# feiyeha/EGM-Unet

Hardware: AMD Instinct MI355X
Metric: train images/sec at 3x512x512 bs=8/GPU (higher is better)
Workload: dtype bf16; 1 GPU; EGM-UNet GRFBUNet(3,2,base_c=32) fwd+5-term-loss+bwd+SGD, 8x3x512x512 per GPU (BASELINE.json configs[1]); global_batch=8, parallelism=dp1, launch=hipGraph replay, world_size=1

## Files before the change

### egm_unet_amd/csrc/blocks.hip

```cpp
#include "common.h"

namespace {

inline int stream_grid(long long total_threads) {
    long long b = (total_threads + 255) / 256;
    if (b > 256 * 16) b = 256 * 16;
    if (b < 1) b = 1;
    return (int)b;
}
__device__ __forceinline__ float sigm(float v) { return 1.f / (1.f + expf(-v)); }

#define PIX_LOOP(total_expr)                                                                           \
    const int ncv = C >> 3;                                                                            \
    const long long total = (total_expr);                                                              \
    for (long long i = blockIdx.x * 256LL + threadIdx.x; i < total; i += (long long)gridDim.x * 256)
#define PIX_LOOP_XCD(total_expr)                                                                       \
    const int ncv = C >> 3;                                                                            \
    const long long total = (total_expr);                                                              \
    for (long long i = xcd_contiguous_item(blockIdx.x, gridDim.x) * 256LL + threadIdx.x; i < total; i += (long long)gridDim.x * 256)

template <typename T>
__global__ void highpass3_kernel(const T* __restrict__ x, int ldx, T* __restrict__ out, int ldo, int N, int H, int W, int C) {
    PIX_LOOP_XCD((long long)N * H * W * ncv) {
        long long p; int cv; egm_divmod(i, ncv, p, cv);
        int xx, yy; egm_pix_yx(p, H, W, yy, xx);
        float s[8], c[8], v[8];
        zero8(s);
        load8(x + p * ldx + cv * 8, c);
#pragma unroll
        for (int r = -1; r <= 1; ++r)
#pragma unroll
            for (int q = -1; q <= 1; ++q) {
                if (yy + r < 0 || yy + r >= H || xx + q < 0 || xx + q >= W) continue;
                load8(x + (p + (long long)r * W + q) * ldx + cv * 8, v);
#pragma unroll
                for (int j = 0; j < 8; ++j) s[j] += v[j];
            }
#pragma unroll
        for (int j = 0; j < 8; ++j) c[j] -= s[j] * (1.f / 9.f);
        store8(out + p * ldo + cv * 8, c);
    }
}

template <typename T>
__global__ void gate_mul_fwd_kernel(const T* __restrict__ x, int ldx, const T* __restrict__ w, int ldw, T* __restrict__ out, int ldo,
                                    long long npix, int C) {
    PIX_LOOP(npix * ncv) {
        long long p; int cv; egm_divmod(i, ncv, p, cv);
        float a[8], b[8];
        load8(x + p * ldx + cv * 8, a); load8(w + p * ldw + cv * 8, b);
#pragma unroll
        for (int j = 0; j < 8; ++j) a[j] *= (1.f + b[j]);
        store8(out + p * ldo + cv * 8, a);
    }
}
template <typename T>
__global__ void gate_mul_bwd_kernel(const T* __restrict__ g, int ldg, const T* __restrict__ x, int ldx, const T* __restrict__ w, int ldw,
                                    T* __restrict__ dx, int lddx, T* __restrict__ dw, int lddw, long long npix, int C) {
    PIX_LOOP(npix * ncv) {
        long long p; int cv; egm_divmod(i, ncv, p, cv);
        float gg[8], a[8], b[8], o1[8], o2[8];
        load8(g + p * ldg + cv * 8, gg); load8(x + p * ldx + cv * 8, a); load8(w + p * ldw + cv * 8, b);
#pragma unroll
        for (int j = 0; j < 8; ++j) { o1[j] = gg[j] * (1.f + b[j]); o2[j] = gg[j] * a[j]; }
        store8(dx + p * lddx + cv * 8, o1); store8(dw + p * lddw + cv * 8, o2);
    }
}

template <typename T>
__global__ void scale_add_relu_fwd_kernel(const T* __restrict__ a, int lda, float alpha, const T* __restrict__ b, int ldb,
                                          T* __restrict__ out, int ldo, long long npix, int C) {
    PIX_LOOP(npix * ncv) {
        long long p; int cv; egm_divmod(i, ncv, p, cv);
        float u[8], v[8];
        load8(a + p * lda + cv * 8, u); load8(b + p * ldb + cv * 8, v);
#pragma unroll
        for (int j = 0; j < 8; ++j) u[j] = fmaxf(fmaf(alpha, u[j], v[j]), 0.f);
        store8(out + p * ldo + cv * 8, u);
    }
}
template <typename T>
__global__ void scale_add_relu_bwd_kernel(const T* __restrict__ g, int ldg, const T* __restrict__ out, int ldo, float alpha,
                                          T* __restrict__ da, int ldda, T* __restrict__ db, int lddb, long long npix, int C) {
    PIX_LOOP(npix * ncv) {
        long long p; int cv; egm_divmod(i, ncv, p, cv);
        float gg[8], o[8], u[8];
        load8(g + p * ldg + cv * 8, gg); load8(out + p * ldo + cv * 8, o);
#pragma unroll
        for (int j = 0; j < 8; ++j) { gg[j] = o[j] > 0.f ? gg[j] : 0.f; u[j] = alpha * gg[j]; }
        store8(da + p * ldda + cv * 8, u); store8(db + p * lddb + cv * 8, gg);
    }
}

template <int GROUP>
// ... 588 lines not shown
        const T v = from_f32<T>(red[((long long)n * 2) * C + c]);
        dst[(long long)n * ldd + c] = v;
        dst[(long long)(N + n) * ldd + c] = v;
    }
}

template <typename T>
__global__ void fold2_pack_kernel(const float* __restrict__ w, float* __restrict__ out, T* __restrict__ wf, T* __restrict__ wd, int rows, int K,
                                  int CoutP, int CinP) {
    for (int i = blockIdx.x * blockDim.x + threadIdx.x; i < CoutP * CinP; i += gridDim.x * blockDim.x) {
        const int co = i / CinP, ci = i - co * CinP;
        float v = 0.f;
        if (co < rows && ci < K) {
            v = w[(long long)co * 2 * K + ci] + w[(long long)co * 2 * K + K + ci];
            out[co * K + ci] = v;
        }
        wf[i] = from_f32<T>(v);
        wd[(long long)ci * CoutP + co] = from_f32<T>(v);
    }
}
template <typename T>
__global__ void merge357_pack_kernel(const float* __restrict__ w3, const float* __restrict__ w5, const float* __restrict__ w7,
                                     const float* __restrict__ b3, const float* __restrict__ b5, const float* __restrict__ b7,
                                     float* __restrict__ w, float* __restrict__ b, T* __restrict__ wf, T* __restrict__ wd, int Co, int Ci,
                                     int CoutP, int CinP) {
    const int total = 49 * CoutP * CinP;
    for (int i = blockIdx.x * blockDim.x + threadIdx.x; i < total; i += gridDim.x * blockDim.x) {
        const int ci = i % CinP, co = (i / CinP) % CoutP, t = i / (CinP * CoutP), r = t / 7, sx = t % 7;
        float v = 0.f;
        if (co < Co && ci < Ci) {
            const int oc = co * Ci + ci;
            v = w7[oc * 49 + t];
            if (r >= 1 && r <= 5 && sx >= 1 && sx <= 5) v += w5[oc * 25 + (r - 1) * 5 + (sx - 1)];
            if (r >= 2 && r <= 4 && sx >= 2 && sx <= 4) v += w3[oc * 9 + (r - 2) * 3 + (sx - 2)];
            w[oc * 49 + t] = v;
        }
        wf[i] = from_f32<T>(v);
        wd[((long long)(48 - t) * CinP + ci) * CoutP + co] = from_f32<T>(v);
        if (i < Co) b[i] = b3[i] + b5[i] + b7[i];
    }
}

}

#define EGM_REQ_VEC(name, ptr, ld, C)                                                                      \
    EGM_REQUIRE((ptr) != nullptr && egm_aligned16(ptr) && (C) > 0 && (C) % 8 == 0 && (ld) >= (C) && (ld) % 8 == 0, \
                name ": bad tensor (ptr/alignment/C=%d/ld=%d)", (int)(C), (int)(ld))
#define EGM_GROUP_SWITCH(G, ...)                                                                \
    switch (G) { case 1: { constexpr int GROUP = 1; __VA_ARGS__; break; } case 2: { constexpr int GROUP = 2; __VA_ARGS__; break; } \
                 case 4: { constexpr int GROUP = 4; __VA_ARGS__; break; } case 8: { constexpr int GROUP = 8; __VA_ARGS__; break; } \
                 case 16: { constexpr int GROUP = 16; __VA_ARGS__; break; } case 32: { constexpr int GROUP = 32; __VA_ARGS__; break; } \
                 default: { constexpr int GROUP = 64; __VA_ARGS__; break; } }

extern "C" int egm_highpass3(int dtype, const void* x, int ldx, void* out, int ldo, int N, int H, int W, int C, egm_stream_t s) {
    EGM_REQ_VEC("highpass3", x, ldx, C); EGM_REQ_VEC("highpass3", out, ldo, C);
    EGM_REQUIRE(N > 0 && H > 0 && W > 0, "highpass3: bad shape");
    EGM_DISPATCH_DTYPE(dtype, hipLaunchKernelGGL((highpass3_kernel<T>), dim3(stream_grid((long long)N * H * W * (C / 8))), dim3(256), 0,
                                                 (hipStream_t)s, (const T*)x, ldx, (T*)out, ldo, N, H, W, C));
    EGM_CHECK_LAUNCH("highpass3");
    return EGM_OK;
}
extern "C" int egm_gate_mul_fwd(int dtype, const void* x, int ldx, const void* w, int ldw, void* out, int ldo, long long npix, int C,
                                egm_stream_t s) {
    EGM_REQ_VEC("gate_mul_fwd", x, ldx, C); EGM_REQ_VEC("gate_mul_fwd", w, ldw, C); EGM_REQ_VEC("gate_mul_fwd", out, ldo, C);
    EGM_DISPATCH_DTYPE(dtype, hipLaunchKernelGGL((gate_mul_fwd_kernel<T>), dim3(stream_grid(npix * (C / 8))), dim3(256), 0, (hipStream_t)s,
                                                 (const T*)x, ldx, (const T*)w, ldw, (T*)out, ldo, npix, C));
    EGM_CHECK_LAUNCH("gate_mul_fwd");
    return EGM_OK;
}
extern "C" int egm_gate_mul_bwd(int dtype, const void* g, int ldg, const void* x, int ldx, const void* w, int ldw, void* dx, int lddx,
                                void* dw, int lddw, long long npix, int C, egm_stream_t s) {
    EGM_REQ_VEC("gate_mul_bwd", g, ldg, C); EGM_REQ_VEC("gate_mul_bwd", x, ldx, C); EGM_REQ_VEC("gate_mul_bwd", w, ldw, C);
    EGM_REQ_VEC("gate_mul_bwd", dx, lddx, C); EGM_REQ_VEC("gate_mul_bwd", dw, lddw, C);
    EGM_DISPATCH_DTYPE(dtype, hipLaunchKernelGGL((gate_mul_bwd_kernel<T>), dim3(stream_grid(npix * (C / 8))), dim3(256), 0, (hipStream_t)s,
                                                 (const T*)g, ldg, (const T*)x, ldx, (const T*)w, ldw, (T*)dx, lddx, (T*)dw, lddw, npix, C));
    EGM_CHECK_LAUNCH("gate_mul_bwd");
    return EGM_OK;
}
extern "C" int egm_scale_add_relu_fwd(int dtype, const void* a, int lda, float alpha, const void* b, int ldb, void* out, int ldo,
                                      long long npix, int C, egm_stream_t s) {
    EGM_REQ_VEC("scale_add_relu_fwd", a, lda, C); EGM_REQ_VEC("scale_add_relu_fwd", b, ldb, C); EGM_REQ_VEC("scale_add_relu_fwd", out, ldo, C);
    EGM_DISPATCH_DTYPE(dtype, hipLaunchKernelGGL((scale_add_relu_fwd_kernel<T>), dim3(stream_grid(npix * (C / 8))), dim3(256), 0,
                                                 (hipStream_t)s, (const T*)a, lda, alpha, (const T*)b, ldb, (T*)out, ldo, npix, C));
    EGM_CHECK_LAUNCH("scale_add_relu_fwd");
    return EGM_OK;
}
extern "C" int egm_scale_add_relu_bwd(int dtype, const void* g, int ldg, const void* out, int ldo, float alpha, void* da, int ldda,
                                      void* db, int lddb, long long npix, int C, egm_stream_t s) {
    EGM_REQ_VEC("scale_add_relu_bwd", g, ldg, C); EGM_REQ_VEC("scale_add_relu_bwd", out, ldo, C);
    EGM_REQ_VEC("scale_add_relu_bwd", da, ldda, C); EGM_REQ_VEC("scale_add_relu_bwd", db, lddb, C);
    EGM_DISPATCH_DTYPE(dtype, hipLaunchKernelGGL((scale_add_relu_bwd_kernel<T>), dim3(stream_grid(npix * (C / 8))), dim3(256), 0,
                                                 (hipStream_t)s, (const T*)g, ldg, (const T*)out, ldo, alpha, (T*)da, ldda, (T*)db, lddb, npix, C));
    EGM_CHECK_LAUNCH("scale_add_relu_bwd");
    return EGM_OK;
}
extern "C" int egm_gate3_fwd(int dtype, const void* x, int ldx, const void* t, int ldt, void* out, int ldo, long long npix, int C,
                             egm_stream_t s) {
    EGM_REQ_VEC("gate3_fwd", x, ldx, C); EGM_REQ_VEC("gate3_fwd", t, ldt, 8); EGM_REQ_VEC("gate3_fwd", out, ldo, C);
    EGM_DISPATCH_DTYPE(dtype, hipLaunchKernelGGL((gate3_fwd_kernel<T>), dim3(stream_grid(npix * (C / 8))), dim3(256), 0, (hipStream_t)s,
                                                 (const T*)x, ldx, (const T*)t, ldt, (T*)out, ldo, npix, C));
    EGM_CHECK_LAUNCH("gate3_fwd");
    return EGM_OK;
}
extern "C" int egm_gate3_bwd(int dtype, const void* g, int ldg, const void* x, int ldx, const void* t, int ldt, void* dx, int lddx,
                             void* dt, int lddt, long long npix, int C, egm_stream_t s) {
    EGM_REQ_VEC("gate3_bwd", g, ldg, C); EGM_REQ_VEC("gate3_bwd", x, ldx, C); EGM_REQ_VEC("gate3_bwd", t, ldt, 8);
    EGM_REQ_VEC("gate3_bwd", dx, lddx, C); EGM_REQ_VEC("gate3_bwd", dt, lddt, 8);
    const int G = group_for(C / 8 > 64 ? 64 : C / 8);
    const int grid = stream_grid(npix * G);
// ... 236 lines not shown
```

### egm_unet_amd/csrc/pool_up.hip

```cpp
#include "common.h"

namespace {

inline int stream_grid(long long total_threads) {
    long long b = (total_threads + 255) / 256;
    if (b > 256 * 16) b = 256 * 16;
    if (b < 1) b = 1;
    return (int)b;
}

template <typename T>
__global__ void nchw_to_nhwc_kernel(const float* __restrict__ src, T* __restrict__ dst, int ld, int N, int C, long long HW) {
    const long long total = (long long)N * HW;
    for (long long i = blockIdx.x * 256LL + threadIdx.x; i < total; i += (long long)gridDim.x * 256) {
        const long long n = i / HW, p = i - n * HW;
        for (int c0 = 0; c0 < ld; c0 += 8) {
            float v[8];
#pragma unroll
            for (int j = 0; j < 8; ++j) v[j] = (c0 + j < C) ? src[(n * C + c0 + j) * HW + p] : 0.f;
            store8(dst + i * ld + c0, v);
        }
    }
}
template <typename T>
__global__ void nhwc_to_nchw_kernel(const T* __restrict__ src, int ld, float* __restrict__ dst, int N, int C, long long HW) {
    const long long total = (long long)N * HW;
    for (long long i = blockIdx.x * 256LL + threadIdx.x; i < total; i += (long long)gridDim.x * 256) {
        const long long n = i / HW, p = i - n * HW;
        for (int c0 = 0; c0 < C; c0 += 8) {
            float v[8];
            load8(src + i * ld + c0, v);
#pragma unroll
            for (int j = 0; j < 8; ++j) if (c0 + j < C) dst[(n * C + c0 + j) * HW + p] = v[j];
        }
    }
}

template <typename T>
__global__ void maxpool2_fwd_kernel(const T* __restrict__ x, int ldx, T* __restrict__ y, int ldy, int N, int H, int W, int C) {
    const int ncv = C >> 3, Ho = H >> 1, Wo = W >> 1;
    const long long total = (long long)N * Ho * Wo * ncv;
    for (long long i = blockIdx.x * 256LL + threadIdx.x; i < total; i += (long long)gridDim.x * 256) {
        long long p; int cv; egm_divmod(i, ncv, p, cv);
        int n, oy, ox; egm_pix_nyx(p, Ho, Wo, n, oy, ox);
        const T* b = x + (((long long)n * H + 2 * oy) * W + 2 * ox) * ldx + cv * 8;
        float a[8], v[8];
        load8(b, a);
        load8(b + ldx, v);
#pragma unroll
        for (int j = 0; j < 8; ++j) a[j] = fmaxf(a[j], v[j]);
        load8(b + (long long)W * ldx, v);
#pragma unroll
        for (int j = 0; j < 8; ++j) a[j] = fmaxf(a[j], v[j]);
// ... 387 lines not shown
        load8(a + p * lda + cv * 8, v);
        load8(b + p * ldb + cv * 8, u);
#pragma unroll
        for (int j = 0; j < 8; ++j) v[j] += u[j];
        load8(c + p * ldc + cv * 8, u);
#pragma unroll
        for (int j = 0; j < 8; ++j) v[j] += u[j];
        if (d != nullptr) {
            load8(d + p * ldd + cv * 8, u);
#pragma unroll
            for (int j = 0; j < 8; ++j) v[j] += u[j];
        }
        store8(out + p * ldo + cv * 8, v);
    }
}
template <typename T>
__global__ void sum4_hp_kernel(const T* __restrict__ a, int lda, const T* __restrict__ b, int ldb, const T* __restrict__ c, int ldc,
                               const T* __restrict__ d, int ldd, T* __restrict__ out, int ldo, int N, int H, int W, int C) {
    const int ncv = C >> 3;
    const long long total = (long long)N * H * W * ncv;
    for (long long i = xcd_contiguous_item(blockIdx.x, gridDim.x) * 256LL + threadIdx.x; i < total; i += (long long)gridDim.x * 256) {
        long long p; int cv; egm_divmod(i, ncv, p, cv);
        int xx, yy; egm_pix_yx(p, H, W, yy, xx);
        float v[8], u[8], s8[8];
        zero8(s8);
        load8(a + p * lda + cv * 8, v);
#pragma unroll
        for (int r = -1; r <= 1; ++r)
#pragma unroll
            for (int q = -1; q <= 1; ++q) {
                if (yy + r < 0 || yy + r >= H || xx + q < 0 || xx + q >= W) continue;
                load8(a + (p + (long long)r * W + q) * lda + cv * 8, u);
#pragma unroll
                for (int j = 0; j < 8; ++j) s8[j] += u[j];
            }
#pragma unroll
        for (int j = 0; j < 8; ++j) v[j] = to_f32(from_f32<T>(v[j] - s8[j] * (1.f / 9.f)));
        load8(b + p * ldb + cv * 8, u);
#pragma unroll
        for (int j = 0; j < 8; ++j) v[j] += u[j];
        if (c != nullptr) {
            load8(c + p * ldc + cv * 8, u);
#pragma unroll
            for (int j = 0; j < 8; ++j) v[j] += u[j];
        }
        if (d != nullptr) {
            load8(d + p * ldd + cv * 8, u);
#pragma unroll
            for (int j = 0; j < 8; ++j) v[j] += u[j];
        }
        store8(out + p * ldo + cv * 8, v);
    }
}
__global__ void vec_add_f32_kernel(float* __restrict__ y, const float* __restrict__ x, long long n) {
    for (long long i = blockIdx.x * 256LL + threadIdx.x; i < n; i += (long long)gridDim.x * 256) y[i] += x[i];
}
__global__ void fill_f32_kernel(float* __restrict__ y, float v, long long n) {
    for (long long i = blockIdx.x * 256LL + threadIdx.x; i < n; i += (long long)gridDim.x * 256) y[i] = v;
}

}

#define EGM_REQ_VEC(name, ptr, ld, C)                                                                      \
    EGM_REQUIRE((ptr) != nullptr && egm_aligned16(ptr) && (C) > 0 && (C) % 8 == 0 && (ld) >= (C) && (ld) % 8 == 0, \
                name ": bad tensor (ptr/alignment/C=%d/ld=%d)", (int)(C), (int)(ld))

extern "C" int egm_nchw_to_nhwc(int dtype, const void* src, void* dst, int ld, int N, int C, int H, int W, egm_stream_t s) {
    EGM_REQUIRE(src && dst && egm_aligned16(dst) && N > 0 && C > 0 && H > 0 && W > 0 && ld >= C && ld % 8 == 0, "nchw_to_nhwc: bad args");
    const long long HW = (long long)H * W;
    EGM_DISPATCH_DTYPE(dtype, hipLaunchKernelGGL((nchw_to_nhwc_kernel<T>), dim3(stream_grid(N * HW)), dim3(256), 0, (hipStream_t)s,
                                                 (const float*)src, (T*)dst, ld, N, C, HW));
    EGM_CHECK_LAUNCH("nchw_to_nhwc");
    return EGM_OK;
}
extern "C" int egm_nhwc_to_nchw(int dtype, const void* src, int ld, void* dst, int N, int C, int H, int W, egm_stream_t s) {
    EGM_REQUIRE(src && dst && egm_aligned16(src) && N > 0 && C > 0 && H > 0 && W > 0 && ld >= C && ld % 8 == 0, "nhwc_to_nchw: bad args");
    const long long HW = (long long)H * W;
    EGM_DISPATCH_DTYPE(dtype, hipLaunchKernelGGL((nhwc_to_nchw_kernel<T>), dim3(stream_grid(N * HW)), dim3(256), 0, (hipStream_t)s,
                                                 (const T*)src, ld, (float*)dst, N, C, HW));
    EGM_CHECK_LAUNCH("nhwc_to_nchw");
    return EGM_OK;
}

extern "C" int egm_maxpool2_fwd(int dtype, const void* x, int ldx, void* y, int ldy, int N, int H, int W, int C, egm_stream_t s) {
    EGM_REQ_VEC("maxpool2_fwd", x, ldx, C);
    EGM_REQ_VEC("maxpool2_fwd", y, ldy, C);
    EGM_REQUIRE(N > 0 && H >= 2 && W >= 2, "maxpool2_fwd: bad shape");
    const long long total = (long long)N * (H / 2) * (W / 2) * (C / 8);
    EGM_DISPATCH_DTYPE(dtype, hipLaunchKernelGGL((maxpool2_fwd_kernel<T>), dim3(stream_grid(total)), dim3(256), 0, (hipStream_t)s,
                                                 (const T*)x, ldx, (T*)y, ldy, N, H, W, C));
    EGM_CHECK_LAUNCH("maxpool2_fwd");
    return EGM_OK;
}
extern "C" int egm_maxpool2_bwd(int dtype, const void* x, int ldx, const void* dy, int lddy, void* dx, int lddx, int N, int H, int W,
                                int C, egm_stream_t s) {
    EGM_REQ_VEC("maxpool2_bwd", x, ldx, C);
    EGM_REQ_VEC("maxpool2_bwd", dy, lddy, C);
    EGM_REQ_VEC("maxpool2_bwd", dx, lddx, C);
    EGM_REQUIRE(N > 0 && H >= 2 && W >= 2, "maxpool2_bwd: bad shape");
    const long long total = (long long)N * (H / 2) * (W / 2) * (C / 8);
    EGM_DISPATCH_DTYPE(dtype, {
        hipLaunchKernelGGL((maxpool2_bwd_kernel<T>), dim3(stream_grid(total)), dim3(256), 0, (hipStream_t)s, (const T*)x, ldx,
                           (const T*)dy, lddy, (const T*)nullptr, 0, (T*)dx, lddx, N, H, W, C);
        if ((H & 1) || (W & 1))
            hipLaunchKernelGGL((zero_tail_kernel<T>), dim3(stream_grid((long long)N * H * W * (C / 8))), dim3(256), 0, (hipStream_t)s,
                               (T*)dx, lddx, N, H, W, C);
    });
    EGM_CHECK_LAUNCH("maxpool2_bwd");
    return EGM_OK;
}

extern "C" int egm_maxpool2_bwd_add(int dtype, const void* x, int ldx, const void* dy, int lddy, const void* add, int ldadd, void* dx, int lddx,
                                    int N, int H, int W, int C, egm_stream_t s) {
    EGM_REQ_VEC("maxpool2_bwd_add", x, ldx, C); EGM_REQ_VEC("maxpool2_bwd_add", dy, lddy, C); EGM_REQ_VEC("maxpool2_bwd_add", add, ldadd, C);
    EGM_REQ_VEC("maxpool2_bwd_add", dx, lddx, C);
    EGM_REQUIRE(N > 0 && H >= 2 && W >= 2 && !(H & 1) && !(W & 1), "maxpool2_bwd_add: H and W must be even (got %d x %d)", H, W);
    const long long total = (long long)N * (H / 2) * (W / 2) * (C / 8);
    EGM_DISPATCH_DTYPE(dtype, hipLaunchKernelGGL((maxpool2_bwd_kernel<T>), dim3(stream_grid(total)), dim3(256), 0, (hipStream_t)s, (const T*)x, ldx,
                                                 (const T*)dy, lddy, (const T*)add, ldadd, (T*)dx, lddx, N, H, W, C));
    EGM_CHECK_LAUNCH("maxpool2_bwd_add");
    return EGM_OK;
}

extern "C" int egm_sum4_hp(int dtype, const void* a, int lda, const void* b, int ldb, const void* c, int ldc, const void* d, int ldd, void* out,
                           int ldo, int N, int H, int W, int C, egm_stream_t s) {
    EGM_REQ_VEC("sum4_hp", a, lda, C); EGM_REQ_VEC("sum4_hp", b, ldb, C); EGM_REQ_VEC("sum4_hp", out, ldo, C);
    if (c != nullptr) EGM_REQ_VEC("sum4_hp", c, ldc, C);
    if (d != nullptr) EGM_REQ_VEC("sum4_hp", d, ldd, C);
    EGM_REQUIRE(N > 0 && H > 0 && W > 0, "sum4_hp: bad shape");
    EGM_DISPATCH_DTYPE(dtype, hipLaunchKernelGGL((sum4_hp_kernel<T>), dim3(stream_grid((long long)N * H * W * (C / 8))), dim3(256), 0, (hipStream_t)s,
                                                 (const T*)a, lda, (const T*)b, ldb, (const T*)c, ldc, (const T*)d, ldd, (T*)out, ldo, N, H, W, C));
    EGM_CHECK_LAUNCH("sum4_hp");
    return EGM_OK;
}
extern "C" int egm_upcat_fwd(int dtype, const void* skip, int lds, const void* low, int ldl, void* out, int ldo, int N, int Hs, int Ws,
                             int Cs, int Hl, int Wl, int Cl, egm_stream_t s) {
    if (skip != nullptr) EGM_REQ_VEC("upcat_fwd", skip, lds, Cs);
    EGM_REQUIRE(Cs > 0 && Cs % 8 == 0, "upcat_fwd: bad Cs %d", Cs);
    EGM_REQ_VEC("upcat_fwd", low, ldl, Cl);
    EGM_REQ_VEC("upcat_fwd", out, ldo, Cs + Cl);
    EGM_REQUIRE(N > 0 && Hl > 0 && Wl > 0 && Hs >= 2 * Hl && Ws >= 2 * Wl, "upcat_fwd: skip must be at least 2x the low-res size");
    const long long total = (long long)N * Hs * Ws * ((skip ? Cs + Cl : Cl) / 8);
    EGM_DISPATCH_DTYPE(dtype, hipLaunchKernelGGL((upcat_fwd_kernel<T>), dim3(stream_grid(total)), dim3(256), 0, (hipStream_t)s,
                                                 (const T*)skip, lds, (const T*)low, ldl, (T*)out, ldo, N, Hs, Ws, Cs, Hl, Wl, Cl));
    EGM_CHECK_LAUNCH("upcat_fwd");
    return EGM_OK;
}
extern "C" int egm_upcat_bwd_low(int dtype, const void* dout, int ldo, void* dlow, int ldl, int N, int Hs, int Ws, int Cs, int Hl,
                                 int Wl, int Cl, egm_stream_t s) {
    EGM_REQ_VEC("upcat_bwd_low", dout, ldo, Cs + Cl);
    EGM_REQ_VEC("upcat_bwd_low", dlow, ldl, Cl);
    EGM_REQUIRE(N > 0 && Hl > 0 && Wl > 0 && Hs >= 2 * Hl && Ws >= 2 * Wl && Cs % 8 == 0, "upcat_bwd_low: bad shape");
    const long long total = (long long)N * Hl * Wl * (Cl / 8);
    if (dtype == EGM_BF16 && Hl >= UB_TY && Wl >= UB_TX) {
        const int tiles_y = egm_cdiv(Hl, UB_TY), tiles_x = egm_cdiv(Wl, UB_TX), nchunk = egm_cdiv(Cl, UB_CB);
        hipLaunchKernelGGL((upcat_bwd_low_tiled_kernel<bf16_t>), dim3((unsigned)((long long)N * tiles_y * tiles_x * nchunk)), dim3(256), 0, (hipStream_t)s,
                           (const bf16_t*)dout, ldo, (bf16_t*)dlow, ldl, N, Hs, Ws, Cs, Hl, Wl, Cl, tiles_x, tiles_y, nchunk);
        EGM_CHECK_LAUNCH("upcat_bwd_low");
        return EGM_OK;
    }
    EGM_DISPATCH_DTYPE(dtype, hipLaunchKernelGGL((upcat_bwd_low_kernel<T>), dim3(stream_grid(total)), dim3(256), 0, (hipStream_t)s,
                                                 (const T*)dout, ldo, (T*)dlow, ldl, N, Hs, Ws, Cs, Hl, Wl, Cl));
    EGM_CHECK_LAUNCH("upcat_bwd_low");
    return EGM_OK;
}

extern "C" int egm_dwconv3_fwd(int dtype, const void* x, int ldx, const float* w, const float* b, const float* scale, void* y, int ldy,
                               int N, int H, int W, int C, egm_stream_t s) {
    EGM_REQ_VEC("dwconv3_fwd", x, ldx, C);
    EGM_REQ_VEC("dwconv3_fwd", y, ldy, C);
    EGM_REQUIRE(w && N > 0 && H > 0 && W > 0, "dwconv3_fwd: bad args");
    const long long total = (long long)N * H * W * (C / 8);
    EGM_DISPATCH_DTYPE(dtype, hipLaunchKernelGGL((dwconv3_fwd_kernel<T>), dim3(stream_grid(total)), dim3(256), (size_t)C * 10 * sizeof(float), (hipStream_t)s,
                                                 (const T*)x, ldx, w, b, scale, (T*)y, ldy, N, H, W, C));
    EGM_CHECK_LAUNCH("dwconv3_fwd");
    return EGM_OK;
}
static int dw_blocks(long long npix, int C) {
    const int rows = 256 / (C >> 3);
    long long b = (npix + rows - 1) / rows;
    if (b > 256) b = 256;
    return (int)(b < 1 ? 1 : b);
// ... 153 lines not shown
```

### include/egm_hip.h

```cpp
#ifndef EGM_HIP_H
#define EGM_HIP_H

#ifdef __cplusplus
extern "C" {
#endif

typedef void* egm_stream_t;

enum egm_status { EGM_OK = 0, EGM_ERR_ARG = -1, EGM_ERR_LAUNCH = -2, EGM_ERR_UNSUPPORTED = -3 };
enum egm_dtype { EGM_F32 = 0, EGM_BF16 = 1 };
enum egm_act { EGM_ACT_NONE = 0, EGM_ACT_RELU = 1, EGM_ACT_SIGMOID = 2, EGM_ACT_SILU = 3  };

int egm_version(void);
const char* egm_last_error(void);
int egm_device_ok(void);

int egm_nchw_to_nhwc(int dtype, const void* src_f32, void* dst, int ld, int N, int C, int H, int W, egm_stream_t s);
int egm_nhwc_to_nchw(int dtype, const void* src, int ld, void* dst_f32, int N, int C, int H, int W, egm_stream_t s);

int egm_conv_pack(int dtype, const void* w_oihw_f32, void* wf, void* wd, int Cout, int Cin, int KH, int KW, int groups,
                  egm_stream_t s);
int egm_conv_pack_chunk(void);
int egm_conv_pack_multi(int dtype, const void* table_dev, int n, long long total_chunks, egm_stream_t s);
int egm_group_begin(void);
// ... 121 lines not shown
int egm_pw_bwd_parts(int dtype, long long npix, int Cin, int CoutTot);
long long egm_pw_bwd_floats(int dtype, long long npix, int Cin, int CoutTot);
int egm_pw_moments(int dtype, const egm_pw_head* heads, int n, egm_stream_t s);
int egm_pw_fwd_coefs(int dtype, const egm_pw_head* heads, int n, egm_stream_t s);
int egm_pw_fwd(int dtype, const egm_pw_head* heads, int n, egm_stream_t s);
int egm_pw_bwd_reduce(int dtype, const egm_pw_head* heads, int n, egm_stream_t s);
int egm_pw_bwd_coefs(int dtype, const egm_pw_head* heads, int n, egm_stream_t s);
int egm_pw_bwd_apply(int dtype, const egm_pw_head* heads, int n, egm_stream_t s);

typedef struct egm_conv1x1_bwd_desc {
    const void* x;  const void* dy;  const void* wd;  void* dx;  float* slabs;
    long long npix;
    int ldx, lddy, lddx, Cin, Cout, pad_;
} egm_conv1x1_bwd_desc;
int egm_conv1x1_bwd_supported(int dtype, int Cin, int Cout);
int egm_conv1x1_bwd_slabs(long long npix);
int egm_conv1x1_bwd(int dtype, const egm_conv1x1_bwd_desc* descs, int n, egm_stream_t s);

int egm_maxpool2_fwd(int dtype, const void* x, int ldx, void* y, int ldy, int N, int H, int W, int C, egm_stream_t s);
int egm_maxpool2_bwd(int dtype, const void* x, int ldx, const void* dy, int lddy, void* dx, int lddx, int N, int H, int W,
                     int C, egm_stream_t s);
int egm_maxpool2_bwd_add(int dtype, const void* x, int ldx, const void* dy, int lddy, const void* add, int ldadd, void* dx, int lddx,
                         int N, int H, int W, int C, egm_stream_t s);
int egm_bn_act_fwd_pool(int dtype, const void* y, int ldy, const float* scale, const float* shift, int act, void* z, int ldz,
                        void* pooled, int ldp, int N, int H, int W, int C, egm_stream_t s);
int egm_bn_pool_bwd_blocks(int N, int H, int W, int C);
int egm_bn_pool_bwd_reduce(int dtype, const void* gskip, int ldgs, const void* gpool, int ldgp, const void* y, int ldy,
                           const float* scale, const float* shift, const float* save_mean, const float* save_rstd, int act,
                           float* partials, int N, int H, int W, int C, egm_stream_t s);
int egm_bn_pool_bwd_apply(int dtype, const void* gskip, int ldgs, const void* gpool, int ldgp, const void* y, int ldy,
                          const float* scale, const float* shift, const float* save_mean, const float* save_rstd, int act, int train,
                          const float* sums, void* dy, int lddy, int N, int H, int W, int C, egm_stream_t s);
int egm_gate3_fwd_pool(int dtype, const void* x, int ldx, const void* t, int ldt, void* out, int ldo, void* pooled, int ldp, int N,
                       int H, int W, int C, egm_stream_t s);
int egm_gate3_pool_bwd(int dtype, const void* gskip, int ldgs, const void* gpool, int ldgp, const void* x, int ldx, const void* t,
                       int ldt, void* dx, int lddx, void* dt, int lddt, int N, int H, int W, int C, egm_stream_t s);
int egm_upcat_fwd(int dtype, const void* skip, int lds, const void* low, int ldl, void* out, int ldo, int N, int Hs, int Ws,
                  int Cs, int Hl, int Wl, int Cl, egm_stream_t s);
int egm_upcat_bwd_low(int dtype, const void* dout, int ldo, void* dlow, int ldl, int N, int Hs, int Ws, int Cs, int Hl,
                      int Wl, int Cl, egm_stream_t s);

int egm_axpby(int dtype, const void* a, int lda, float alpha, const void* b, int ldb, float beta, void* out, int ldo,
              long long npix, int C, egm_stream_t s);
int egm_sum4(int dtype, const void* a, int lda, const void* b, int ldb, const void* c, int ldc, const void* d, int ldd, void* out,
             int ldo, long long npix, int C, egm_stream_t s);
int egm_sum4_hp(int dtype, const void* a, int lda, const void* b, int ldb, const void* c, int ldc, const void* d, int ldd, void* out,
                int ldo, int N, int H, int W, int C, egm_stream_t s);
int egm_vec_add_f32(float* y, const float* x, long long n, egm_stream_t s);
int egm_fill_f32(float* y, float v, long long n, egm_stream_t s);
int egm_copy_cols_f32(const float* src, int ld_src, int col0_src, float* dst, int ld_dst, int col0_dst, int rows, int ncols,
                      egm_stream_t s);

int egm_highpass3(int dtype, const void* x, int ldx, void* out, int ldo, int N, int H, int W, int C, egm_stream_t s);
int egm_gate_mul_fwd(int dtype, const void* x, int ldx, const void* w, int ldw, void* out, int ldo, long long npix, int C,
                     egm_stream_t s);
int egm_gate_mul_bwd(int dtype, const void* g, int ldg, const void* x, int ldx, const void* w, int ldw, void* dx, int lddx,
                     void* dw, int lddw, long long npix, int C, egm_stream_t s);

int egm_scale_add_relu_fwd(int dtype, const void* a, int lda, float alpha, const void* b, int ldb, void* out, int ldo,
                           long long npix, int C, egm_stream_t s);
int egm_scale_add_relu_bwd(int dtype, const void* g, int ldg, const void* out, int ldo, float alpha, void* da, int ldda,
                           void* db, int lddb, long long npix, int C, egm_stream_t s);
int egm_gate3_fwd(int dtype, const void* x, int ldx, const void* t, int ldt, void* out, int ldo, long long npix, int C,
                  egm_stream_t s);
int egm_gate3_bwd(int dtype, const void* g, int ldg, const void* x, int ldx, const void* t, int ldt, void* dx, int lddx,
                  void* dt, int lddt, long long npix, int C, egm_stream_t s);

int egm_bcast_gate_fwd(int dtype, const void* a, int lda, const void* gl, int ldgl, void* out, int ldo, long long npix, int C,
                       egm_stream_t s);
int egm_bcast_gate_bwd(int dtype, const void* g, int ldg, const void* a, int lda, const void* gl, int ldgl, void* da, int ldda,
                       void* dgl, int lddgl, long long npix, int C, egm_stream_t s);
int egm_gelu_fwd(int dtype, const void* x, int ldx, void* out, int ldo, long long npix, int C, egm_stream_t s);
int egm_gelu_bwd(int dtype, const void* g, int ldg, const void* x, int ldx, void* dx, int lddx, long long npix, int C,
                 egm_stream_t s);

int egm_chan_meanmax_fwd(int dtype, const void* x, int ldx, void* out, int ldo, long long npix, int C, int C_real,
                         egm_stream_t s);
int egm_chan_meanmax_bwd(int dtype, const void* g, int ldg, const void* x, int ldx, void* dx, int lddx, long long npix, int C,
                         int C_real, egm_stream_t s);
int egm_sa_conv7_fwd(int dtype, const void* x, int ldx, const float* w, void* y, int ldy, int N, int H, int W, egm_stream_t s);
long long egm_sa_conv7_bwd_workspace(int N, int H, int W);
int egm_sa_conv7_bwd(int dtype, const void* x, int ldx, const void* dy, int lddy, const float* w, void* dx, int lddx, float* dw,
                     void* workspace, int N, int H, int W, egm_stream_t s);
long long egm_global_pool_workspace(int N, long long HW, int C);
int egm_global_avgmax_fwd(int dtype, const void* x, int ldx, void* out, int* argidx, void* workspace, int N, long long HW,
                          int C, egm_stream_t s);
int egm_global_avgmax_bwd(int dtype, const void* gout, const int* argidx, void* dx, int lddx, int N, long long HW, int C,
                          egm_stream_t s);
int egm_rows_dup(int dtype, const float* red, void* dst, int ldd, int N, int C, egm_stream_t s);
int egm_ca_mlp_fwd(int dtype, const void* pooled, int ldp, const float* w0, const float* w2, float* h, void* logits, int ldo, int R,
                   int C, int Cr, egm_stream_t s);
int egm_ca_mlp_bwd(int dtype, const void* dlogits, int ldd, const void* pooled, int ldp, const float* h, const float* w0,
                   const float* w2, float* dw0, float* dw2, void* dpooled, int lddp, int R, int C, int Cr, egm_stream_t s);
int egm_fusion_combine_fwd(int dtype, const void* f, int ldf, const void* sv, int lds, const void* sa, int ldsa, const void* ca,
                           void* out, int ldo, int N, long long HW, int C, egm_stream_t s);
int egm_fusion_combine_blocks(long long HW, int C);
int egm_fusion_combine_bwd(int dtype, const void* g, int ldg, const void* sv, int lds, const void* sa, int ldsa, const void* ca,
                           void* ds, int ldds, void* dsa, int lddsa, float* partials, int N, long long HW, int C, egm_stream_t s);
int egm_fold2_fwd(const float* w, float* out, int rows, int K, egm_stream_t s);
int egm_fold2_bwd(const float* g, float* dw, int rows, int K, egm_stream_t s);
int egm_merge357_fwd(const float* w3, const float* w5, const float* w7, const float* b3, const float* b5, const float* b7,
                     float* w, float* b, int Co, int Ci, egm_stream_t s);
int egm_merge357_bwd(const float* gw, float* d3, float* d5, float* d7, const float* gb, float* gb3, int Co, int Ci, egm_stream_t s);
int egm_fold2_pack(int dtype, const float* w, float* out, void* wf, void* wd, int rows, int K, egm_stream_t s);
int egm_merge357_pack(int dtype, const float* w3, const float* w5, const float* w7, const float* b3, const float* b5, const float* b7,
                      float* w, float* b, void* wf, void* wd, int Co, int Ci, egm_stream_t s);
// ... 168 lines not shown
```

Before: 684.4 images/s.

## Add row-marching LDS ring-buffer stencil kernels for bf16 highpass3 and sum4_hp

Adds a shared stencil3 header that implements the 3x3 box-highpass as a vertical march. Each block owns a strip of columns and a band of rows, keeps a 4-row LDS ring, prefetches upcoming rows into registers, and shares horizontal neighbours through LDS. This replaces the old per-pixel kernel, which reloaded all 9 neighbours from global memory. Both highpass3 and sum4_hp (fused highpass plus fan-in adds, specialised per fan-in) use it for large bf16 tensors, with an env/API knob to disable it or force the band size. The cost is a per-row block barrier, register pressure from deep prefetch, and recomputed halo columns.

Result: no change. 687.1 images/s (median of 6 runs) (+0.4%).

```diff
diff --git a/egm_unet_amd/csrc/blocks.hip b/egm_unet_amd/csrc/blocks.hip
--- a/egm_unet_amd/csrc/blocks.hip
+++ b/egm_unet_amd/csrc/blocks.hip
@@ -1,4 +1,6 @@
 #include "common.h"
+#include <stdlib.h>
+#include "stencil3.h"
 
 namespace {
 
@@ -40,6 +42,12 @@
         for (int j = 0; j < 8; ++j) c[j] -= s[j] * (1.f / 9.f);
         store8(out + p * ldo + cv * 8, c);
     }
+}
+
+__global__ void __launch_bounds__(stencil3::kThreads)
+highpass3_march_kernel(const bf16_t* __restrict__ x, int ldx, bf16_t* __restrict__ out, int ldo, int N, int H, int W, int C, int CH, int TXL,
+                       int TY) {
+    stencil3::march<0>(x, ldx, nullptr, 0, nullptr, 0, nullptr, 0, out, ldo, N, H, W, C, CH, TXL, TY);
 }
 
 template <typename T>
@@ -734,9 +742,29 @@
                  case 16: { constexpr int GROUP = 16; __VA_ARGS__; break; } case 32: { constexpr int GROUP = 32; __VA_ARGS__; break; } \
                  default: { constexpr int GROUP = 64; __VA_ARGS__; break; } }
 
+static int g_stencil_mode = -1, g_stencil_rows = 0;
+extern "C" int egm_stencil_mode(int mode) {
+    if (g_stencil_mode < 0) g_stencil_mode = getenv("EGM_STENCIL_MODE") ? atoi(getenv("EGM_STENCIL_MODE")) & 3 : 1;
+    const int old = g_stencil_mode;
+    if (mode >= 0) g_stencil_mode = mode & 3;
+    return old;
+}
+extern "C" int egm_stencil_rows(int rows) {
+    const int old = g_stencil_rows;
+    if (rows >= 0 && rows <= stencil3::kMaxForcedRows) g_stencil_rows = rows;
+    return old;
+}
+
 extern "C" int egm_highpass3(int dtype, const void* x, int ldx, void* out, int ldo, int N, int H, int W, int C, egm_stream_t s) {
     EGM_REQ_VEC("highpass3", x, ldx, C); EGM_REQ_VEC("highpass3", out, ldo, C);
     EGM_REQUIRE(N > 0 && H > 0 && W > 0, "highpass3: bad shape");
+    stencil3::Plan pl;
+    if (stencil3::plan(egm_stencil_mode(-1), egm_stencil_rows(-1), dtype, N, H, W, C, pl)) {
+        hipLaunchKernelGGL(highpass3_march_kernel, dim3(pl.blocks), dim3(stencil3::kThreads), 0, (hipStream_t)s, (const bf16_t*)x, ldx,
+                           (bf16_t*)out, ldo, N, H, W, C, pl.CH, pl.TXL, pl.TY);
+        EGM_CHECK_LAUNCH("highpass3");
+        return EGM_OK;
+    }
     EGM_DISPATCH_DTYPE(dtype, hipLaunchKernelGGL((highpass3_kernel<T>), dim3(stream_grid((long long)N * H * W * (C / 8))), dim3(256), 0,
                                                  (hipStream_t)s, (const T*)x, ldx, (T*)out, ldo, N, H, W, C));
     EGM_CHECK_LAUNCH("highpass3");
diff --git a/egm_unet_amd/csrc/pool_up.hip b/egm_unet_amd/csrc/pool_up.hip
--- a/egm_unet_amd/csrc/pool_up.hip
+++ b/egm_unet_amd/csrc/pool_up.hip
@@ -1,4 +1,5 @@
 #include "common.h"
+#include "stencil3.h"
 
 namespace {
 
@@ -492,6 +493,13 @@
         store8(out + p * ldo + cv * 8, v);
     }
 }
+template <int FAN>
+__global__ void __launch_bounds__(stencil3::kThreads)
+sum4_hp_march_kernel(const bf16_t* __restrict__ a, int lda, const bf16_t* __restrict__ b, int ldb, const bf16_t* __restrict__ c, int ldc,
+                     const bf16_t* __restrict__ d, int ldd, bf16_t* __restrict__ out, int ldo, int N, int H, int W, int C, int CH, int TXL,
+                     int TY) {
+    stencil3::march<FAN>(a, lda, b, ldb, c, ldc, d, ldd, out, ldo, N, H, W, C, CH, TXL, TY);
+}
 __global__ void vec_add_f32_kernel(float* __restrict__ y, const float* __restrict__ x, long long n) {
     for (long long i = blockIdx.x * 256LL + threadIdx.x; i < n; i += (long long)gridDim.x * 256) y[i] += x[i];
 }
@@ -568,6 +576,22 @@
     if (c != nullptr) EGM_REQ_VEC("sum4_hp", c, ldc, C);
     if (d != nullptr) EGM_REQ_VEC("sum4_hp", d, ldd, C);
     EGM_REQUIRE(N > 0 && H > 0 && W > 0, "sum4_hp: bad shape");
+    stencil3::Plan pl;
+    if (stencil3::plan(egm_stencil_mode(-1), egm_stencil_rows(-1), dtype, N, H, W, C, pl)) {
+#define EGM_SUM4_HP_MARCH(FAN)                                                                                                       \
+        hipLaunchKernelGGL((sum4_hp_march_kernel<FAN>), dim3(pl.blocks), dim3(stencil3::kThreads), 0, (hipStream_t)s, (const bf16_t*)a, \
+                           lda, (const bf16_t*)b, ldb, (const bf16_t*)c, ldc, (const bf16_t*)d, ldd, (bf16_t*)out, ldo, N, H, W, C,     \
+                           pl.CH, pl.TXL, pl.TY)
+        switch ((c != nullptr ? 2 : 0) | (d != nullptr ? 4 : 0)) {
+            case 0: EGM_SUM4_HP_MARCH(1); break;
+            case 2: EGM_SUM4_HP_MARCH(3); break;
+            case 4: EGM_SUM4_HP_MARCH(5); break;
+            default: EGM_SUM4_HP_MARCH(7); break;
+        }
+#undef EGM_SUM4_HP_MARCH
+        EGM_CHECK_LAUNCH("sum4_hp");
+        return EGM_OK;
+    }
     EGM_DISPATCH_DTYPE(dtype, hipLaunchKernelGGL((sum4_hp_kernel<T>), dim3(stream_grid((long long)N * H * W * (C / 8))), dim3(256), 0, (hipStream_t)s,
                                                  (const T*)a, lda, (const T*)b, ldb, (const T*)c, ldc, (const T*)d, ldd, (T*)out, ldo, N, H, W, C));
     EGM_CHECK_LAUNCH("sum4_hp");
diff --git a/egm_unet_amd/csrc/stencil3.h b/egm_unet_amd/csrc/stencil3.h
--- /dev/null
+++ b/egm_unet_amd/csrc/stencil3.h
@@ -0,0 +1,169 @@
+#pragma once
+#include <type_traits>
+#include "common.h"
+
+namespace stencil3 {
+
+constexpr int kThreads = 256;
+constexpr int kMaxChunk = 8;
+constexpr int kRing = 4;
+#ifndef EGM_STENCIL_DEPTH
+#define EGM_STENCIL_DEPTH 8
+#endif
+#ifndef EGM_STENCIL_FAN_DEPTH
+#define EGM_STENCIL_FAN_DEPTH 4
+#endif
+constexpr int kFanLead = 3, kFanBufs = 4;
+constexpr int kRows[] = {24, 16, 8};
+constexpr int kMaxForcedRows = 64;
+constexpr long long kMinBytes = 32ll << 20;
+
+struct Plan { int CH, TXL, TY, blocks; };
+
+static inline long long items(int N, int H, int W, int C, int TY) {
+    const int ncv = C >> 3, CH = ncv < kMaxChunk ? ncv : kMaxChunk, TXL = kThreads / CH;
+    return (long long)N * egm_cdiv(H, TY) * egm_cdiv(W, TXL - 2) * egm_cdiv(ncv, CH);
+}
+static inline bool plan(int mode, int rows, int dtype, int N, int H, int W, int C, Plan& p) {
+    if (dtype != EGM_BF16 || !(mode & 1)) return false;
+    if (!(mode & 2) && (long long)N * H * W * C * 2 < kMinBytes) return false;
+    int TY = rows;
+    if (rows <= 0)
+        for (int t : kRows) {
+            TY = t;
+            if (items(N, H, W, C, TY) >= 4 * 256) break;
+        }
+    const long long n = items(N, H, W, C, TY);
+    if (n > (1ll << 30)) return false;
+    const int ncv = C >> 3;
+    p.CH = ncv < kMaxChunk ? ncv : kMaxChunk; p.TXL = kThreads / p.CH; p.TY = TY; p.blocks = (int)n;
+    return true;
+}
+
+__device__ __forceinline__ void unpack8(const uint4& a, float (&v)[8]) {
+    v[0] = __uint_as_float(a.x << 16); v[1] = __uint_as_float(a.x & 0xffff0000u);
+    v[2] = __uint_as_float(a.y << 16); v[3] = __uint_as_float(a.y & 0xffff0000u);
+    v[4] = __uint_as_float(a.z << 16); v[5] = __uint_as_float(a.z & 0xffff0000u);
+    v[6] = __uint_as_float(a.w << 16); v[7] = __uint_as_float(a.w & 0xffff0000u);
+}
+__device__ __forceinline__ void add8(float (&s)[8], const uint4& a) {
+    float u[8];
+    unpack8(a, u);
+#pragma unroll
+    for (int j = 0; j < 8; ++j) s[j] += u[j];
+}
+__device__ __forceinline__ uint4 ldg16(const bf16_t* p) { return *reinterpret_cast<const uint4*>(p); }
+
+template <int FAN>
+__device__ __forceinline__ void march(const bf16_t* __restrict__ x, int ldx, const bf16_t* __restrict__ b, int ldb,
+                                      const bf16_t* __restrict__ c, int ldc, const bf16_t* __restrict__ d, int ldd,
+                                      bf16_t* __restrict__ out, int ldo, int N, int H, int W, int C, int CH, int TXL, int TY) {
+    constexpr int kDepth = FAN ? EGM_STENCIL_FAN_DEPTH : EGM_STENCIL_DEPTH;
+    static_assert(kDepth % kFanBufs == 0 && kDepth >= 4, "groups of kDepth steps index the prefetch registers statically");
+    __shared__ uint4 ring[kRing][kThreads];
+    const int ncv = C >> 3, TXO = TXL - 2;
+    const int nchunk = (ncv + CH - 1) / CH, nstrip = (W + TXO - 1) / TXO, nband = (H + TY - 1) / TY;
+    int item = xcd_contiguous_item(blockIdx.x, gridDim.x);
+    const int chunk = item % nchunk; item /= nchunk;
+    const int strip = item % nstrip; item /= nstrip;
+    const int band = item % nband;
+    const int n = item / nband;
+
+    const int tid = threadIdx.x, px = tid / CH, cvl = tid - px * CH, cv = chunk * CH + cvl;
+    const int xx = strip * TXO - 1 + px, y0 = band * TY;
+    const int rows = H - y0 < TY ? H - y0 : TY;
+    const bool in_ok = px < TXL && cv < ncv && xx >= 0 && xx < W;
+    const bool out_ok = in_ok && px >= 1 && px <= TXO;
+    const int xc = xx < 0 ? 0 : xx >= W ? W - 1 : xx, cvc = cv < ncv ? cv : ncv - 1;
+    const long long img = (long long)n * H * W;
+    const bf16_t* xcol = x + (img + xc) * ldx + cvc * 8;
+    const long long xrow = (long long)W * ldx;
+    bf16_t* ocol = out + (img + xc) * ldo + cvc * 8;
+    const uint4 zero = make_uint4(0u, 0u, 0u, 0u);
+
+    auto row_clamped = [&](int yi) { return yi < 0 ? 0 : yi >= H ? H - 1 : yi; };
+    auto row_value = [&](int yi, const uint4& v) { return in_ok && yi >= 0 && yi < H ? v : zero; };
+    const bf16_t* bcol = (FAN & 1) ? b + (img + xc) * ldb + cvc * 8 : nullptr;
+    const bf16_t* ccol = (FAN & 2) ? c + (img + xc) * ldc + cvc * 8 : nullptr;
+    const bf16_t* dcol = (FAN & 4) ? d + (img + xc) * ldd + cvc * 8 : nullptr;
+    auto load_fan = [&](int y, uint4& vb, uint4& vc, uint4& vd) {
+        const long long r = (long long)row_clamped(y) * W;
+        if (FAN & 1) vb = ldg16(bcol + r * ldb);
+        if (FAN & 2) vc = ldg16(ccol + r * ldc);
+        if (FAN & 4) vd = ldg16(dcol + r * ldd);
+    };
+
+    uint4 pf[kDepth];
+#pragma unroll
+    for (int k = 0; k < kDepth; ++k) pf[k] = ldg16(xcol + row_clamped(y0 - 1 + k) * xrow);
+    uint4 fb[kFanBufs], fc[kFanBufs], fd[kFanBufs];
+#pragma unroll
+    for (int k = 0; k < kFanLead; ++k) load_fan(y0 + k, fb[k], fc[k], fd[k]);
+    const uint4 r0 = row_value(y0 - 1, pf[0]), r1 = row_value(y0, pf[1]);
+    ring[0][tid] = r0; ring[1][tid] = r1;
+    pf[0] = ldg16(xcol + row_clamped(y0 - 1 + kDepth) * xrow);
+    pf[1] = ldg16(xcol + row_clamped(y0 + kDepth) * xrow);
+    uint4 cm = zero, c0 = r0, cp = r1;
+    const int lcell = tid >= CH ? tid - CH : tid, rcell = tid + CH < kThreads ? tid + CH : tid;
+
+    auto group = [&](auto more_tag, int tb) {
+        constexpr bool MORE = decltype(more_tag)::value;
+#pragma unroll
+        for (int k = 0; k < kDepth; ++k) {
+            const int t = tb + k;
+            if (!MORE && t >= rows) break;
+            const int slot = (k + 2) % kDepth;
+            const uint4 v = row_value(y0 + 1 + t, pf[slot]);
+            ring[(t + 2) & (kRing - 1)][tid] = v;
+            if (MORE) pf[slot] = ldg16(xcol + row_clamped(y0 + 1 + t + kDepth) * xrow);
+            cm = c0; c0 = cp; cp = v;
+            const int fl = (k + kFanLead) % kFanBufs;
+            if (FAN && (MORE || k + kFanLead < kDepth)) load_fan(y0 + t + kFanLead, fb[fl], fc[fl], fd[fl]);
+            asm volatile("s_waitcnt lgkmcnt(0)" ::: "memory");
+            __builtin_amdgcn_s_barrier();
+            float s[8], cc[8];
+            zero8(s);
+#pragma unroll
+            for (int r = 0; r < 3; ++r) {
+                const uint4* row = ring[(t + r) & (kRing - 1)];
+                add8(s, row[lcell]);
+                add8(s, r == 0 ? cm : r == 1 ? c0 : cp);
+                add8(s, row[rcell]);
+            }
+            unpack8(c0, cc);
+            if (FAN) {
+                float u[8];
+#pragma unroll
+                for (int i = 0; i < 8; ++i) cc[i] = to_f32(from_f32<bf16_t>(cc[i] - s[i] * (1.f / 9.f)));
+                unpack8(fb[k % kFanBufs], u);
+#pragma unroll
+                for (int i = 0; i < 8; ++i) cc[i] += u[i];
+                if (FAN & 2) {
+                    unpack8(fc[k % kFanBufs], u);
+#pragma unroll
+                    for (int i = 0; i < 8; ++i) cc[i] += u[i];
+                }
+                if (FAN & 4) {
+                    unpack8(fd[k % kFanBufs], u);
+#pragma unroll
+                    for (int i = 0; i < 8; ++i) cc[i] += u[i];
+                }
+            } else {
+#pragma unroll
+                for (int i = 0; i < 8; ++i) cc[i] -= s[i] * (1.f / 9.f);
+            }
+            egm_u32x4 o;
+            o.x = (uint32_t)f32_to_bf16(cc[0]) | ((uint32_t)f32_to_bf16(cc[1]) << 16);
+            o.y = (uint32_t)f32_to_bf16(cc[2]) | ((uint32_t)f32_to_bf16(cc[3]) << 16);
+            o.z = (uint32_t)f32_to_bf16(cc[4]) | ((uint32_t)f32_to_bf16(cc[5]) << 16);
+            o.w = (uint32_t)f32_to_bf16(cc[6]) | ((uint32_t)f32_to_bf16(cc[7]) << 16);
+            bf16_t* dst = ocol + (long long)(y0 + t) * W * ldo;
+            if (out_ok) egm_store16_as<EGM_STORE_MODE>(dst, o);
+        }
+    };
+    int tb = 0;
+    for (; tb + kDepth < rows; tb += kDepth) group(std::true_type{}, tb);
+    group(std::false_type{}, tb);
+}
+
+}
diff --git a/include/egm_hip.h b/include/egm_hip.h
--- a/include/egm_hip.h
+++ b/include/egm_hip.h
@@ -197,6 +197,8 @@
                       egm_stream_t s);
 
 int egm_highpass3(int dtype, const void* x, int ldx, void* out, int ldo, int N, int H, int W, int C, egm_stream_t s);
+int egm_stencil_mode(int mode);
+int egm_stencil_rows(int rows);
 int egm_gate_mul_fwd(int dtype, const void* x, int ldx, const void* w, int ldw, void* out, int ldo, long long npix, int C,
                      egm_stream_t s);
 int egm_gate_mul_bwd(int dtype, const void* g, int ldg, const void* x, int ldx, const void* w, int ldw, void* dx, int lddx,
```
